# davidbau/rewriting

Hardware: NVIDIA H100
Metric: StyleGAN2-256 images/sec (higher is better)
Workload: dtype bf16x3 (3-term split bf16 operands, fp32 accumulate; fp32 in/out)

## Files before the change

### rewriting_b200/csrc/conv_tc.cu

```cuda
#include <cstdlib>
#include <cstring>

#include "rw_common.cuh"
#include "rw_kernels.h"

namespace rw {

namespace {

constexpr int BM = 128;
constexpr int BK = 32;
constexpr int MMA_K = 16;
constexpr int kStages = 7;
constexpr int kNumThreads = 384;
constexpr int kTmaWarp = 8;
constexpr uint32_t kProducerRegs = 40;
constexpr uint32_t kConsumerRegs = 232;
constexpr int kCluster = 2;
constexpr int kChunkKB = 16;

template <int BN>
struct ConvSmem {
  static constexpr int kABytes = BM * BK * 2;
  static constexpr int kBBytes = BN * BK * 2;
// ... 35 lines not shown

  const int m_tiles = (p.rows + BM - 1) / BM;
  const int n_tiles = p.Cout / BN;
  const int mn_units = (m_tiles + kCluster - 1) / kCluster * n_tiles;
  const int num_units = mn_units * p.nphase;
  const int kb_per_tap = p.Cin / BK;

  if (warp == kTmaWarp && lane == 0) {
    tma_prefetch_desc(&map_a_hi);
    tma_prefetch_desc(&map_a_lo);
    tma_prefetch_desc(&map_w_hi);
    tma_prefetch_desc(&map_w_lo);
    for (int s = 0; s < kStages; ++s) {
      mbar_init(&bars->full[s], 1);
      mbar_init(&bars->empty[s], 2 * kCluster);
    }
    fence_mbar_init();
  }
  cluster_sync();

  if (warp < kTmaWarp) {
    setmaxnreg_inc<kConsumerRegs>();
    const int wg = threadIdx.x >> 7;
    const int c = lane & 3;
    const int img = p.Hp * p.Wp;
    auto release = [&](int s) {
      if ((threadIdx.x & 127) == 0) {
#pragma unroll
        for (int r = 0; r < kCluster; ++r) mbar_arrive_cluster(mapa_shared(&bars->empty[s], r));
      }
    };
    auto clk = [] { return static_cast<uint32_t>(clock()); };
    uint32_t prof[6] = {0, 0, 0, 0, 0, 0};
    uint32_t tp0 = 0, tp1 = 0;
    if constexpr (PROF) prof[5] = 0u - clk();
    int stage = 0;
    uint32_t phase = 0;
    for (int unit = first_unit; unit < num_units; unit += nsched) {
      int ph, mn;
      decode_tile(unit, p.nphase, nsched, ph, mn);
      const int num_kb = p.ph_ntaps[ph] * kb_per_tap;
      const int n_tile = mn % n_tiles;
      const int n0 = n_tile * BN;
      const int m0 = ((mn / n_tiles) * kCluster + rank) * BM;

      float acc[NR], d[NR];
#pragma unroll
      for (int j = 0; j < NR; ++j) acc[j] = 0.f;
      for (int kb0 = 0; kb0 < num_kb; kb0 += kChunkKB) {
        const int kb_end = (kb0 + kChunkKB < num_kb) ? kb0 + kChunkKB : num_kb;
        int held = -1;
        for (int kb = kb0; kb < kb_end; ++kb) {
          if constexpr (PROF) tp0 = clk();
          mbar_wait(&bars->full[stage], phase);
          if constexpr (PROF) { tp1 = clk(); prof[0] += tp1 - tp0; }
          const uint32_t sa = smem_u32(smem + stage * S::kStageBytes);
          const uint64_t da_hi = make_smem_desc(sa + wg * (S::kABytes / 2), 16, 512, 2);
          const uint64_t da_lo = make_smem_desc(sa + S::kABytes + wg * (S::kABytes / 2), 16, 512, 2);
          const uint64_t db_hi = make_smem_desc(sa + 2 * S::kABytes, 16, 512, 2);
          const uint64_t db_lo = make_smem_desc(sa + 2 * S::kABytes + S::kBBytes, 16, 512, 2);
          wgmma_fence();
#pragma unroll
          for (int kk = 0; kk < BK / MMA_K; ++kk) {
            const uint64_t adv = static_cast<uint64_t>((kk * MMA_K * 2) >> 4);
            wgmma_m64nN<0, 0>(d, da_lo + adv, db_hi + adv, ((kb - kb0) | kk) != 0);
            wgmma_m64nN<0, 0>(d, da_hi + adv, db_lo + adv, 1u);
            wgmma_m64nN<0, 0>(d, da_hi + adv, db_hi + adv, 1u);
          }
          wgmma_commit();
          wgmma_wait<1>();
          if (held >= 0) release(held);
          held = stage;
          if (++stage == kStages) { stage = 0; phase ^= 1u; }
          if constexpr (PROF) prof[1] += clk() - tp1;
        }
        if constexpr (PROF) tp0 = clk();
        wgmma_wait<0>();
        release(held);
#pragma unroll
        for (int j = 0; j < NR; ++j) acc[j] += d[j];
        if constexpr (PROF) prof[2] += clk() - tp0;
      }
      if constexpr (PROF) tp0 = clk();

      uint32_t tid;
      asm volatile("mov.u32 %0, %%tid.x;\n" : "=r"(tid));
      const int row0 = m0 + ((tid >> 7) << 6) + (((tid >> 5) & 3) << 4) + ((tid & 31) >> 2);
#pragma unroll
      for (int i = 0; i < 2; ++i) {
        const int prow = row0 + 8 * i;
        const int b = prow / img;
        const int rem = prow - b * img;
        const int yy = rem / p.Wp;
        const int xx = rem - yy * p.Wp;
        const int Hv = p.ph_Hv[ph], Wv = p.ph_Wv[ph];
        const bool in_rows = prow < p.rows;
        const bool valid = in_rows && (yy < Hv) && (xx < Wv);
        const float* scl = (p.scale_bo && in_rows) ? p.scale_bo + static_cast<size_t>(b) * p.Cout : nullptr;
        float* outp = (p.out != nullptr && p.out_mode == 0 && valid)
                          ? p.out + p.ph_out_ofs[ph] + static_cast<size_t>(b) * p.out_sb +
                                static_cast<size_t>(yy) * p.out_sy + static_cast<size_t>(xx) * p.out_sx
                          : nullptr;
        if (EPI == 1 || !valid) {
          if (scl && (EPI == 1 || p.out_mode == 1)) {
#pragma unroll
            for (int j = 0; j < NJ; ++j) {
              const float2 sv = __ldg(reinterpret_cast<const float2*>(scl + n0 + 8 * j + 2 * c));
              acc[4 * j + 2 * i] *= sv.x;
              acc[4 * j + 2 * i + 1] *= sv.y;
            }
          }
          if (EPI == 1 && outp) {
#pragma unroll
            for (int j = 0; j < NJ; ++j)
#pragma unroll
              for (int e = 0; e < 2; ++e)
                outp[static_cast<size_t>(n0 + 8 * j + 2 * c + e) * p.out_sc] = acc[4 * j + 2 * i + e];
          }
        } else {
          float nz = 0.f;
          if (p.noise != nullptr)
            nz = __ldg(p.noise_w) * __ldg(p.noise + static_cast<size_t>(b) * p.noise_bstride +
                                          static_cast<size_t>(yy) * Wv + xx);
          const float act_gain = p.act_gain != 0.f ? p.act_gain : 1.4142135623730951f;
          if (scl) {
            const float* sc = scl + n0 + 2 * c;
#pragma unroll
            for (int j = 0; j < NJ; ++j)
#pragma unroll
              for (int e = 0; e < 2; ++e) acc[4 * j + 2 * i + e] *= __ldg(sc + 8 * j + e);
// ... 239 lines not shown
```

### rewriting_b200/csrc/rw_common.cuh

```cuda
#pragma once
#include <cuda_runtime.h>
#include <cuda_bf16.h>
#include <cuda.h>
#include <stdint.h>

namespace rw {

enum : int {
  RW_OK = 0,
  RW_ERR_BAD_ARG = -1,
  RW_ERR_CUDA = -2,
  RW_ERR_NO_DRIVER_SYMBOL = -3,
  RW_ERR_UNSUPPORTED = -4,
};
void set_last_error(const char* fmt, ...);
int check_cuda(cudaError_t e, const char* what);

#ifndef RW_SPIN_LIMIT
#define RW_SPIN_LIMIT (1u << 26)
#endif

__device__ __forceinline__ uint32_t smem_u32(const void* p) {
  return static_cast<uint32_t>(__cvta_generic_to_shared(p));
}

__device__ __forceinline__ uint32_t lane_id() { return threadIdx.x & 31u; }

__device__ __forceinline__ bool elect_one() {
  uint32_t pred = 0;
  asm volatile(
      "{\n\t.reg .pred P;\n\t"
      "elect.sync _|P, 0xffffffff;\n\t"
      "selp.u32 %0, 1, 0, P;\n\t}\n"
      : "=r"(pred));
  return pred != 0;
}

__device__ __forceinline__ void mbar_init(uint64_t* bar, uint32_t count) {
  asm volatile("mbarrier.init.shared::cta.b64 [%0], %1;\n" ::"r"(smem_u32(bar)), "r"(count));
}
__device__ __forceinline__ void fence_mbar_init() {
  asm volatile("fence.mbarrier_init.release.cluster;\n" ::: "memory");
}
__device__ __forceinline__ void fence_proxy_async_smem() {
  asm volatile("fence.proxy.async.shared::cta;\n" ::: "memory");
}
__device__ __forceinline__ void mbar_expect_tx(uint64_t* bar, uint32_t bytes) {
  asm volatile("mbarrier.arrive.expect_tx.shared::cta.b64 _, [%0], %1;\n" ::"r"(smem_u32(bar)),
               "r"(bytes)
               : "memory");
}
__device__ __forceinline__ void mbar_arrive(uint64_t* bar) {
  asm volatile("mbarrier.arrive.shared::cta.b64 _, [%0];\n" ::"r"(smem_u32(bar)) : "memory");
}
__device__ __forceinline__ bool mbar_try_wait(uint64_t* bar, uint32_t parity) {
  uint32_t ok;
  asm volatile(
      "{\n\t.reg .pred P;\n\t"
      "mbarrier.try_wait.parity.shared::cta.b64 P, [%1], %2;\n\t"
      "selp.u32 %0, 1, 0, P;\n\t}\n"
      : "=r"(ok)
      : "r"(smem_u32(bar)), "r"(parity)
      : "memory");
  return ok != 0;
}
__device__ __forceinline__ void mbar_wait(uint64_t* bar, uint32_t parity) {
  uint32_t spins = 0;
  while (!mbar_try_wait(bar, parity)) {
    if (++spins > RW_SPIN_LIMIT) __trap();
  }
}
__device__ __forceinline__ void named_bar_sync(int id, int count) {
  asm volatile("bar.sync %0, %1;\n" ::"r"(id), "r"(count) : "memory");
}

__device__ __forceinline__ uint32_t cluster_ctarank() {
  uint32_t r;
  asm volatile("mov.u32 %0, %%cluster_ctarank;\n" : "=r"(r));
  return r;
}
__device__ __forceinline__ uint32_t cluster_id_x() {
  uint32_t r;
  asm volatile("mov.u32 %0, %%clusterid.x;\n" : "=r"(r));
  return r;
}
__device__ __forceinline__ uint32_t num_clusters_x() {
  uint32_t r;
  asm volatile("mov.u32 %0, %%nclusterid.x;\n" : "=r"(r));
  return r;
}
__device__ __forceinline__ void cluster_sync() {
  asm volatile("barrier.cluster.arrive.release;\nbarrier.cluster.wait.acquire;\n" ::: "memory");
}
__device__ __forceinline__ uint32_t mapa_shared(const void* p, uint32_t rank) {
  uint32_t r;
  asm volatile("mapa.shared::cluster.u32 %0, %1, %2;\n" : "=r"(r) : "r"(smem_u32(p)), "r"(rank));
  return r;
}
__device__ __forceinline__ void mbar_arrive_cluster(uint32_t cluster_addr) {
  asm volatile("mbarrier.arrive.shared::cluster.b64 _, [%0];\n" ::"r"(cluster_addr) : "memory");
}

template <uint32_t N>
__device__ __forceinline__ void setmaxnreg_dec() {
  asm volatile("setmaxnreg.dec.sync.aligned.u32 %0;\n" ::"n"(N));
}
template <uint32_t N>
__device__ __forceinline__ void setmaxnreg_inc() {
  asm volatile("setmaxnreg.inc.sync.aligned.u32 %0;\n" ::"n"(N));
}

__device__ __forceinline__ void tma_prefetch_desc(const CUtensorMap* m) {
  asm volatile("prefetch.tensormap [%0];\n" ::"l"(reinterpret_cast<uint64_t>(m)) : "memory");
}
__device__ __forceinline__ void tma_load_2d(void* smem_dst, const CUtensorMap* m, uint64_t* bar,
                                            int32_t c_inner, int32_t c_outer) {
  asm volatile(
      "cp.async.bulk.tensor.2d.shared::cluster.global.mbarrier::complete_tx::bytes"
      " [%0], [%1, {%3, %4}], [%2];\n" ::"r"(smem_u32(smem_dst)),
      "l"(reinterpret_cast<uint64_t>(m)), "r"(smem_u32(bar)), "r"(c_inner), "r"(c_outer)
      : "memory");
}
__device__ __forceinline__ void tma_load_2d_multicast(void* smem_dst, const CUtensorMap* m,
                                                      uint64_t* bar, int32_t c_inner,
                                                      int32_t c_outer, uint16_t cta_mask) {
  asm volatile(
      "cp.async.bulk.tensor.2d.shared::cluster.global.mbarrier::complete_tx::bytes.multicast::cluster"
      " [%0], [%1, {%3, %4}], [%2], %5;\n" ::"r"(smem_u32(smem_dst)),
      "l"(reinterpret_cast<uint64_t>(m)), "r"(smem_u32(bar)), "r"(c_inner), "r"(c_outer),
      "h"(cta_mask)
      : "memory");
}

__device__ __forceinline__ void wgmma_fence() {
  asm volatile("wgmma.fence.sync.aligned;\n" ::: "memory");
}
__device__ __forceinline__ void wgmma_commit() {
  asm volatile("wgmma.commit_group.sync.aligned;\n" ::: "memory");
}
template <int N>
__device__ __forceinline__ void wgmma_wait() {
  asm volatile("wgmma.wait_group.sync.aligned %0;\n" ::"n"(N) : "memory");
}
template <int TA, int TB>
__device__ __forceinline__ void wgmma_m64n128(float (&d)[64], uint64_t desc_a, uint64_t desc_b,
                                               uint32_t accumulate) {
  asm volatile(
      "{\n\t.reg .pred p;\n\t"
      "setp.ne.b32 p, %66, 0;\n\t"
      "wgmma.mma_async.sync.aligned.m64n128k16.f32.bf16.bf16 "
      "{%0, %1, %2, %3, %4, %5, %6, %7, %8, %9, %10, %11, %12, %13, %14, %15, %16, %17, %18, %19, %20, %21, %22, %23, %24, %25, %26, %27, %28, %29, %30, %31, %32, %33, %34, %35, %36, %37, %38, %39, %40, %41, %42, %43, %44, %45, %46, %47, %48, %49, %50, %51, %52, %53, %54, %55, %56, %57, %58, %59, %60, %61, %62, %63}, "
      "%64, %65, p, 1, 1, %67, %68;\n\t}\n"
      : "+f"(d[0]), "+f"(d[1]), "+f"(d[2]), "+f"(d[3]), "+f"(d[4]), "+f"(d[5]), "+f"(d[6]), "+f"(d[7]),
        "+f"(d[8]), "+f"(d[9]), "+f"(d[10]), "+f"(d[11]), "+f"(d[12]), "+f"(d[13]), "+f"(d[14]), "+f"(d[15]),
        "+f"(d[16]), "+f"(d[17]), "+f"(d[18]), "+f"(d[19]), "+f"(d[20]), "+f"(d[21]), "+f"(d[22]), "+f"(d[23]),
        "+f"(d[24]), "+f"(d[25]), "+f"(d[26]), "+f"(d[27]), "+f"(d[28]), "+f"(d[29]), "+f"(d[30]), "+f"(d[31]),
        "+f"(d[32]), "+f"(d[33]), "+f"(d[34]), "+f"(d[35]), "+f"(d[36]), "+f"(d[37]), "+f"(d[38]), "+f"(d[39]),
        "+f"(d[40]), "+f"(d[41]), "+f"(d[42]), "+f"(d[43]), "+f"(d[44]), "+f"(d[45]), "+f"(d[46]), "+f"(d[47]),
        "+f"(d[48]), "+f"(d[49]), "+f"(d[50]), "+f"(d[51]), "+f"(d[52]), "+f"(d[53]), "+f"(d[54]), "+f"(d[55]),
        "+f"(d[56]), "+f"(d[57]), "+f"(d[58]), "+f"(d[59]), "+f"(d[60]), "+f"(d[61]), "+f"(d[62]), "+f"(d[63])
      : "l"(desc_a), "l"(desc_b), "r"(accumulate), "n"(TA), "n"(TB));
}
template <int TA, int TB>
__device__ __forceinline__ void wgmma_m64n64(float (&d)[32], uint64_t desc_a, uint64_t desc_b,
                                              uint32_t accumulate) {
  asm volatile(
      "{\n\t.reg .pred p;\n\t"
      "setp.ne.b32 p, %34, 0;\n\t"
      "wgmma.mma_async.sync.aligned.m64n64k16.f32.bf16.bf16 "
      "{%0, %1, %2, %3, %4, %5, %6, %7, %8, %9, %10, %11, %12, %13, %14, %15, %16, %17, %18, %19, %20, %21, %22, %23, %24, %25, %26, %27, %28, %29, %30, %31}, "
      "%32, %33, p, 1, 1, %35, %36;\n\t}\n"
      : "+f"(d[0]), "+f"(d[1]), "+f"(d[2]), "+f"(d[3]), "+f"(d[4]), "+f"(d[5]), "+f"(d[6]), "+f"(d[7]),
        "+f"(d[8]), "+f"(d[9]), "+f"(d[10]), "+f"(d[11]), "+f"(d[12]), "+f"(d[13]), "+f"(d[14]), "+f"(d[15]),
        "+f"(d[16]), "+f"(d[17]), "+f"(d[18]), "+f"(d[19]), "+f"(d[20]), "+f"(d[21]), "+f"(d[22]), "+f"(d[23]),
        "+f"(d[24]), "+f"(d[25]), "+f"(d[26]), "+f"(d[27]), "+f"(d[28]), "+f"(d[29]), "+f"(d[30]), "+f"(d[31])
      : "l"(desc_a), "l"(desc_b), "r"(accumulate), "n"(TA), "n"(TB));
}
template <int TA, int TB, int NR>
__device__ __forceinline__ void wgmma_m64nN(float (&d)[NR], uint64_t desc_a, uint64_t desc_b,
                                             uint32_t accumulate) {
  static_assert(NR == 64 || NR == 32, "wgmma_m64nN: N = 128 or 64");
  if constexpr (NR == 64) wgmma_m64n128<TA, TB>(d, desc_a, desc_b, accumulate);
  else wgmma_m64n64<TA, TB>(d, desc_a, desc_b, accumulate);
}
template <int TA, int TB>
__device__ __forceinline__ void wgmma_m64n144(float (&d)[72], uint64_t desc_a, uint64_t desc_b,
                                               uint32_t accumulate) {
  asm volatile(
      "{\n\t.reg .pred p;\n\t"
      "setp.ne.b32 p, %74, 0;\n\t"
      "wgmma.mma_async.sync.aligned.m64n144k16.f32.bf16.bf16 "
      "{%0, %1, %2, %3, %4, %5, %6, %7, %8, %9, %10, %11, %12, %13, %14, %15, %16, %17, %18, %19, %20, %21, %22, %23, %24, %25, %26, %27, %28, %29, %30, %31, %32, %33, %34, %35, %36, %37, %38, %39, %40, %41, %42, %43, %44, %45, %46, %47, %48, %49, %50, %51, %52, %53, %54, %55, %56, %57, %58, %59, %60, %61, %62, %63, %64, %65, %66, %67, %68, %69, %70, %71}, "
      "%72, %73, p, 1, 1, %75, %76;\n\t}\n"
      : "+f"(d[0]), "+f"(d[1]), "+f"(d[2]), "+f"(d[3]), "+f"(d[4]), "+f"(d[5]), "+f"(d[6]), "+f"(d[7]),
        "+f"(d[8]), "+f"(d[9]), "+f"(d[10]), "+f"(d[11]), "+f"(d[12]), "+f"(d[13]), "+f"(d[14]), "+f"(d[15]),
// ... 35 lines not shown
```

### rewriting_b200/csrc/upconv_tc.cu

```cuda
#include <cstring>

#include "rw_common.cuh"
#include "rw_kernels.h"

namespace rw {

namespace {

constexpr int UM = 128;
constexpr int UNC = 16;
constexpr int UN = 9 * UNC;
constexpr int UBK = 32;
constexpr int UK = 16;
constexpr int kUStages = 5;
constexpr int kUThreads = 384;
constexpr int kUTmaWarp = 8;
constexpr uint32_t kUProducerRegs = 40;
constexpr uint32_t kUConsumerRegs = 232;
constexpr int kUABytes = UM * UBK * 2;
constexpr int kUBBytes = UN * UBK * 2;
constexpr int kUStageBytes = 2 * kUABytes + 2 * kUBBytes;
constexpr int kUMailFloats = 2 * 2 * 4 * 2 * 32;
constexpr int kUOutSlotBytes = 64 * 32;
constexpr int kUOutQuarterBytes = 2 * kUOutSlotBytes;
constexpr int kUOutStageBytes = 4 * kUOutQuarterBytes;
constexpr int kUXchgFloat2 = 9 * 2 * 32;
constexpr int kUXchgBytes = 8 * kUXchgFloat2 * 8;
constexpr int kUSmemTotal =
    kUStages * kUStageBytes + kUMailFloats * 4 + kUOutStageBytes + kUXchgBytes + 512 + 256;
static_assert(kUSmemTotal <= 232448, "upconv_fused: shared memory over the per-block limit");

struct UBarriers {
  uint64_t full[kUStages];
  uint64_t empty[kUStages];
};

__device__ __forceinline__ void tma_load_5d(void* smem_dst, const CUtensorMap* m, uint64_t* bar,
                                            int32_t c0, int32_t c1, int32_t c2, int32_t c3,
                                            int32_t c4) {
  asm volatile(
      "cp.async.bulk.tensor.5d.shared::cluster.global.mbarrier::complete_tx::bytes"
      " [%0], [%1, {%3, %4, %5, %6, %7}], [%2];\n" ::"r"(smem_u32(smem_dst)),
      "l"(reinterpret_cast<uint64_t>(m)), "r"(smem_u32(bar)), "r"(c0), "r"(c1), "r"(c2), "r"(c3),
      "r"(c4)
      : "memory");
}

__device__ __forceinline__ float2 f2add(float2 a, float2 b) {
  return make_float2(__fadd_rn(a.x, b.x), __fadd_rn(a.y, b.y));
}
__device__ __forceinline__ float2 f2mul(float2 a, float2 b) {
  return make_float2(__fmul_rn(a.x, b.x), __fmul_rn(a.y, b.y));
}
__device__ __forceinline__ float2 f2fma(float2 a, float2 b, float2 c) {
  return make_float2(__fmaf_rn(a.x, b.x, c.x), __fmaf_rn(a.y, b.y, c.y));
}
__device__ __forceinline__ void mbar_wait_relaxed(uint64_t* bar, uint32_t parity) {
  uint32_t spins = 0;
  while (!mbar_try_wait(bar, parity)) {
    __nanosleep(40);
    if (++spins > RW_SPIN_LIMIT) __trap();
  }
}

__device__ __forceinline__ void sts_v4(uint32_t a, float x, float y, float z, float w) {
  asm volatile("st.shared.v4.f32 [%0], {%1, %2, %3, %4};\n" ::"r"(a), "f"(x), "f"(y), "f"(z), "f"(w)
               : "memory");
}
__device__ __forceinline__ void lds_v4(uint32_t a, float& x, float& y, float& z, float& w) {
  asm volatile("ld.shared.v4.f32 {%0, %1, %2, %3}, [%4];\n"
               : "=f"(x), "=f"(y), "=f"(z), "=f"(w)
               : "r"(a)
               : "memory");
}

constexpr int kBarPair = 3;
template <int N>
__device__ __forceinline__ void tma_store_wait_read_n() {
  asm volatile("cp.async.bulk.wait_group.read %0;\n" ::"n"(N) : "memory");
}

struct UpItem {
  int bg, band, cg;
  int y_first, y_emit, y_end;
};

__device__ __forceinline__ UpItem decode_item(int item, const UpFusedParams& p) {
  UpItem it;
  it.cg = item % p.ncg;
  const int r = item / p.ncg;
  it.band = r % p.nbands;
  it.bg = r / p.nbands;
  const int ya = 1 + (it.band * p.H) / p.nbands;
  const int yb = 1 + ((it.band + 1) * p.H) / p.nbands;
  it.y_emit = ya;
  it.y_first = ya - 2 < 0 ? 0 : ya - 2;
  it.y_end = yb;
  return it;
}

__device__ __forceinline__ void stmatrix_x4(uint32_t addr, const uint32_t (&r)[4]) {
  asm volatile("stmatrix.sync.aligned.m8n8.x4.shared.b16 [%0], {%1, %2, %3, %4};\n" ::"r"(addr),
               "r"(r[0]), "r"(r[1]), "r"(r[2]), "r"(r[3])
               : "memory");
}

__device__ __forceinline__ void tma_store_5d(const CUtensorMap* m, uint32_t smem_src, int32_t c0,
                                             int32_t c1, int32_t c2, int32_t c3, int32_t c4) {
  asm volatile(
      "cp.async.bulk.tensor.5d.global.shared::cta.bulk_group [%0, {%2, %3, %4, %5, %6}], [%1];\n" ::"l"(
          reinterpret_cast<uint64_t>(m)),
      "r"(smem_src), "r"(c0), "r"(c1), "r"(c2), "r"(c3), "r"(c4)
      : "memory");
  asm volatile("cp.async.bulk.commit_group;\n" ::: "memory");
}
__device__ __forceinline__ void tma_store_wait_all() {
  asm volatile("cp.async.bulk.wait_group 0;\n" ::: "memory");
}

template <bool PROF, bool NCHW>
__global__ void __launch_bounds__(kUThreads, 1)
upconv_fused_kernel(const __grid_constant__ CUtensorMap map_a_hi,
                    const __grid_constant__ CUtensorMap map_a_lo,
                    const __grid_constant__ CUtensorMap map_w_hi,
                    const __grid_constant__ CUtensorMap map_w_lo,
                    const __grid_constant__ CUtensorMap map_o_hi,
                    const __grid_constant__ CUtensorMap map_o_lo, const UpFusedParams p) {
  extern __shared__ uint8_t smem_raw[];
  uint8_t* smem = reinterpret_cast<uint8_t*>((reinterpret_cast<uintptr_t>(smem_raw) + 511) &
                                             ~static_cast<uintptr_t>(511));
  float* mail = reinterpret_cast<float*>(smem + kUStages * kUStageBytes);
  uint8_t* out_stage = smem + kUStages * kUStageBytes + kUMailFloats * 4;
  float2* xchg = reinterpret_cast<float2*>(out_stage + kUOutStageBytes);
  UBarriers* bars = reinterpret_cast<UBarriers*>(out_stage + kUOutStageBytes + kUXchgBytes);

  const int warp = __shfl_sync(0xffffffffu, static_cast<int>(threadIdx.x >> 5), 0);
  const int lane = threadIdx.x & 31;
  const int kb_count = p.Cin / UBK;
  const int G = UM / p.W;

  if (warp == kUTmaWarp && lane == 0) {
    tma_prefetch_desc(&map_a_hi);
    tma_prefetch_desc(&map_a_lo);
    tma_prefetch_desc(&map_w_hi);
    tma_prefetch_desc(&map_w_lo);
    tma_prefetch_desc(&map_o_hi);
    tma_prefetch_desc(&map_o_lo);
    for (int s = 0; s < kUStages; ++s) {
      mbar_init(&bars->full[s], 1);
      mbar_init(&bars->empty[s], 2);
    }
    fence_mbar_init();
  }
  __syncthreads();

  if (warp < kUTmaWarp) {
    setmaxnreg_inc<kUConsumerRegs>();
    const int wg = warp >> 2;
    const int q = warp >> 1;
    const int h = warp & 1;
    int stage = 0;
    uint32_t phase = 0;
    const int g = lane >> 2, c = lane & 3;
    const int W = p.W;
    const int T0 = q * 32 + 4 * g;
    const int x0 = T0 & (W - 1);
    const int img_in_tile = T0 / W;
    const int Ho = 2 * p.H, Wo = 2 * W;
    const bool first_x = (x0 == 0), last_x = (x0 + 4 == W);
    const bool cross = W > 32;
    const bool mail_l = cross && g == 0 && !first_x, mail_r = cross && g == 7 && !last_x;
    float kv[4], kh[4];
    {
      const float k00 = __ldg(p.k4 + 15);
#pragma unroll
      for (int a = 0; a < 4; ++a) {
        kv[a] = __ldg(p.k4 + 15 - a * 4);
        kh[a] = __ldg(p.k4 + 15 - a) / k00;
      }
    }
    const float nw = (!NCHW || (p.noise != nullptr && p.noise_w != nullptr)) ? __ldg(p.noise_w) : 0.f;
    uint32_t step = 0;
    constexpr uint32_t kMailBufBytes = 2 * 4 * 2 * 32 * 4;
    const uint32_t mail_s = smem_u32(mail) + h * (4 * 2 * 32 * 4) + c * 32;
    const uint32_t post_r = mail_s + (q * 2 + 1) * 128, post_l = mail_s + (q * 2 + 0) * 128;
    const uint32_t read_l = mail_s + ((q - 1) * 2 + 1) * 128, read_r = mail_s + ((q + 1) * 2 + 0) * 128;
    const uint32_t slot_s = smem_u32(out_stage) + q * kUOutQuarterBytes;
    uint32_t st_addr[2];
    {
      const int m = lane >> 3, gp = lane & 7;
      const int Wm = W < 32 ? W : 32;
      const int tl = 4 * gp + m;
      const int il = tl / W;
      const int xg = ((4 * gp) & (Wm - 1)) >> 2;
#pragma unroll
      for (int xi = 0; xi < 2; ++xi) {
        uint32_t a = slot_s + (((il * 8 + 2 * m + xi) * (Wm >> 2) + xg) << 5) + (h << 4);
        a ^= ((a >> 7) & 1u) << 4;
        st_addr[xi] = a;
      }
    }
    const CUtensorMap* omap = h ? &map_o_lo : &map_o_hi;
    const uint32_t my_slot = slot_s + h * kUOutSlotBytes;
    const int o_xg = ((32 * q) & (W - 1)) >> 2;
    const int o_img = (32 * q) / W;
    long long prof_acc[16] = {0, 0, 0, 0, 0, 0, 0, 0, 0, 0, 0, 0, 0, 0, 0, 0};

    for (int item = blockIdx.x; item < p.nitems; item += gridDim.x) {
      const UpItem it = decode_item(item, p);
      const int b0 = it.bg * G;
      const int b = b0 + img_in_tile;
      const bool img_ok = b < p.B;
      const int c0 = it.cg * UNC + h * 8 + 2 * c;
      const size_t chan_o = static_cast<size_t>(img_ok ? b : 0) * p.Cout + c0;
      float2 dm = make_float2(1.f, 1.f), bs = make_float2(0.f, 0.f), ns = make_float2(1.f, 1.f);
      if (!NCHW || p.demod != nullptr) dm = __ldg(reinterpret_cast<const float2*>(p.demod + chan_o));
      if (!NCHW || (p.act && p.bias != nullptr)) bs = __ldg(reinterpret_cast<const float2*>(p.bias + c0));
      if (!NCHW) ns = __ldg(reinterpret_cast<const float2*>(p.next_scale + chan_o));
      const bool has_noise = !NCHW || (p.noise != nullptr && p.noise_w != nullptr);
      float2 c20[4], c21[4], c22[4];
      float2 w0[2][4], w1[2][4], w2[2][4];
#pragma unroll
      for (int j = 0; j < 4; ++j) {
        c20[j] = c21[j] = c22[j] = make_float2(0.f, 0.f);
        w0[0][j] = w0[1][j] = w1[0][j] = w1[1][j] = w2[0][j] = w2[1][j] = make_float2(0.f, 0.f);
      }
      const float* nrow_base = p.noise + static_cast<size_t>(img_ok ? b : 0) * p.noise_bstride + 2 * x0;
      __nv_bfloat16* out_hi = static_cast<__nv_bfloat16*>(p.next_hi);
      __nv_bfloat16* out_lo = static_cast<__nv_bfloat16*>(p.next_lo);
      const size_t img_row0 = static_cast<size_t>(img_ok ? b : 0) * (Ho + 1);

      for (int y = it.y_first; y < it.y_end; ++y, ++step) {
        const bool rows_out = (y >= it.y_emit);
        const bool emit = rows_out && img_ok;
        if (emit && c < 2 && has_noise) {
          const float* np = nrow_base + static_cast<size_t>(2 * y - 2 + c) * Wo;
          asm volatile("prefetch.global.L1 [%0];\n" ::"l"(np));
        }
        long long tq[8];
        if constexpr (PROF) tq[0] = clock64();
        float2 P[9][4];
        {
          float d[72];
          int held = -1;
          for (int kb = 0; kb < kb_count; ++kb) {
            mbar_wait(&bars->full[stage], phase);
            const uint32_t sa = smem_u32(smem + stage * kUStageBytes);
            const uint64_t da_hi = make_smem_desc(sa + wg * (kUABytes / 2), 16, 512, 2);
            const uint64_t da_lo = make_smem_desc(sa + kUABytes + wg * (kUABytes / 2), 16, 512, 2);
            const uint64_t db_hi = make_smem_desc(sa + 2 * kUABytes, 16, 512, 2);
            const uint64_t db_lo = make_smem_desc(sa + 2 * kUABytes + kUBBytes, 16, 512, 2);
            wgmma_fence();
#pragma unroll
            for (int kk = 0; kk < UBK / UK; ++kk) {
              const uint64_t adv = static_cast<uint64_t>((kk * UK * 2) >> 4);
              wgmma_m64n144<0, 0>(d, da_lo + adv, db_hi + adv, (kb | kk) != 0);
              wgmma_m64n144<0, 0>(d, da_hi + adv, db_lo + adv, 1u);
              wgmma_m64n144<0, 0>(d, da_hi + adv, db_hi + adv, 1u);
            }
            wgmma_commit();
            wgmma_wait<1>();
            if (held >= 0 && (threadIdx.x & 127) == 0) mbar_arrive(&bars->empty[held]);
            held = stage;
            if (++stage == kUStages) { stage = 0; phase ^= 1u; }
          }
          wgmma_wait<0>();
          if ((threadIdx.x & 127) == 0) mbar_arrive(&bars->empty[held]);
          if constexpr (PROF) tq[1] = clock64();
          float2* to = xchg + (warp ^ 1) * kUXchgFloat2 + lane;
#pragma unroll
          for (int t = 0; t < 9; ++t)
#pragma unroll
            for (int i = 0; i < 2; ++i)
              to[(t * 2 + i) * 32] = h ? make_float2(d[4 * t + 2 * i], d[4 * t + 2 * i + 1])
                                       : make_float2(d[4 * (9 + t) + 2 * i], d[4 * (9 + t) + 2 * i + 1]);
          named_bar_sync(kBarPair + q, 64);
          const float2* from = xchg + warp * kUXchgFloat2 + lane;
#pragma unroll
          for (int t = 0; t < 9; ++t)
#pragma unroll
            for (int i = 0; i < 2; ++i) {
              const float2 own = h ? make_float2(d[4 * (9 + t) + 2 * i], d[4 * (9 + t) + 2 * i + 1])
                                   : make_float2(d[4 * t + 2 * i], d[4 * t + 2 * i + 1]);
              const float2 other = from[(t * 2 + i) * 32];
              P[t][i] = h ? other : own;
              P[t][2 + i] = h ? own : other;
            }
          named_bar_sync(kBarPair + q, 64);
        }
        if constexpr (PROF) tq[2] = clock64();
        if (p.debug_p != nullptr && img_ok && y < p.H && y >= it.y_emit - 1) {
#pragma unroll
          for (int j = 0; j < 4; ++j) {
            float* dp = p.debug_p + ((static_cast<size_t>(b) * p.H + y) * W + x0 + j) * 9 * p.Cout + c0;
#pragma unroll
            for (int t = 0; t < 9; ++t) *reinterpret_cast<float2*>(dp + t * p.Cout) = P[t][j];
          }
        }

        float2 le[2][4], ro[2][4], od[2][4];
#pragma unroll
        for (int j = 0; j < 4; ++j) {
          le[0][j] = f2add(P[0][j], c20[j]);
          od[0][j] = f2add(P[1][j], c21[j]);
          ro[0][j] = f2add(P[2][j], c22[j]);
          le[1][j] = P[3][j];
          od[1][j] = P[4][j];
          ro[1][j] = P[5][j];
          c20[j] = P[6][j];
          c21[j] = P[7][j];
          c22[j] = P[8][j];
        }
        const uint32_t mbo = (step & 1u) * kMailBufBytes;
        if (cross) {
          if (g == 7) {
            sts_v4(post_r + mbo, ro[0][3].x, ro[0][3].y, od[0][3].x, od[0][3].y);
            sts_v4(post_r + mbo + 16, ro[1][3].x, ro[1][3].y, od[1][3].x, od[1][3].y);
          }
          if (g == 0) {
            sts_v4(post_l + mbo, le[0][0].x, le[0][0].y, od[0][0].x, od[0][0].y);
// ... 75 lines not shown
                const float nzv = nw * nz[2 * j + xi];
                float2 v;
                if (yi == 0)
                  v = f2fma(kv3, hf[0][xi][j],
                                 f2fma(kv2, w2[xi][j], f2fma(kv1, w1[xi][j], f2mul(kv0, w0[xi][j]))));
                else
                  v = f2fma(kv3, hf[1][xi][j],
                                 f2fma(kv2, hf[0][xi][j], f2fma(kv1, w2[xi][j], f2mul(kv0, w1[xi][j]))));
                v = f2add(f2fma(v, dm, make_float2(nzv, nzv)), bs);
                if (!NCHW || p.act) {
                  const float2 t02 = f2mul(v, make_float2(0.2f, 0.2f));
                  v = f2mul(make_float2(fmaxf(v.x, t02.x), fmaxf(v.y, t02.y)),
                                 make_float2(1.4142135623730951f, 1.4142135623730951f));
                }
                if constexpr (NCHW) {
                  yv[xi][j] = v;
                } else {
                  const float2 kk = f2mul(ns, v);
                  const __nv_bfloat162 hh = __floats2bfloat162_rn(kk.x, kk.y);
                  const uint32_t hu = *reinterpret_cast<const uint32_t*>(&hh);
                  const __nv_bfloat162 ll = __floats2bfloat162_rn(
                      kk.x - __uint_as_float(hu << 16), kk.y - __uint_as_float(hu & 0xffff0000u));
                  hw[xi][j] = hu;
                  lw[xi][j] = *reinterpret_cast<const uint32_t*>(&ll);
                }
              }
            }
            if constexpr (NCHW) {
              if (img_ok) {
                float* yrow = p.y_out + ((static_cast<size_t>(b) * p.Cout + c0) * Ho + Y) * Wo + 2 * x0;
                const size_t cstride = static_cast<size_t>(Ho) * Wo;
                *reinterpret_cast<float4*>(yrow) = make_float4(yv[0][0].x, yv[1][0].x, yv[0][1].x, yv[1][1].x);
                *reinterpret_cast<float4*>(yrow + 4) = make_float4(yv[0][2].x, yv[1][2].x, yv[0][3].x, yv[1][3].x);
                *reinterpret_cast<float4*>(yrow + cstride) = make_float4(yv[0][0].y, yv[1][0].y, yv[0][1].y, yv[1][1].y);
                *reinterpret_cast<float4*>(yrow + cstride + 4) =
                    make_float4(yv[0][2].y, yv[1][2].y, yv[0][3].y, yv[1][3].y);
              }
              continue;
            }
            if constexpr (PROF) te[1] = clock64();
            if (lane == 0) tma_store_wait_read_n<0>();
            named_bar_sync(kBarPair + q, 64);
            if constexpr (PROF) te[2] = clock64();
#pragma unroll
            for (int xi = 0; xi < 2; ++xi) {
              stmatrix_x4(st_addr[xi], hw[xi]);
              stmatrix_x4(st_addr[xi] + kUOutSlotBytes, lw[xi]);
            }
            if constexpr (PROF) te[5] = clock64();
            fence_proxy_async_smem();
            if constexpr (PROF) te[6] = clock64();
            named_bar_sync(kBarPair + q, 64);
            if constexpr (PROF) te[3] = clock64();
            if (lane == 0 && (!PROF || p.debug_nostore == 0))
              tma_store_5d(omap, my_slot, it.cg * UNC, o_xg, 0, Y, b0 + o_img);
            if constexpr (PROF) {
              te[4] = clock64();
#pragma unroll
              for (int i = 0; i < 4; ++i) prof_acc[8 + i] += te[i + 1] - te[i];
              prof_acc[12] += te[5] - te[2];
              prof_acc[13] += te[6] - te[5];
              prof_acc[14] += te[3] - te[6];
            }
            if (img_ok && last_x && c == 0) {
              const size_t off = ((img_row0 + Y) * (Wo + 1) + Wo) * p.Cout + it.cg * UNC + h * 8;
              *reinterpret_cast<uint4*>(out_hi + off) = make_uint4(0u, 0u, 0u, 0u);
              *reinterpret_cast<uint4*>(out_lo + off) = make_uint4(0u, 0u, 0u, 0u);
            }
          }
        }
        if (!NCHW && emit && y == p.H) {
          const size_t prow = (img_row0 + Ho) * (Wo + 1);
#pragma unroll
          for (int i = 0; i < 3; ++i) {
            if (i < 2 || (last_x && c == 3)) {
              const size_t off = (prow + 2 * x0 + 2 * c + i) * p.Cout + it.cg * UNC + h * 8;
              *reinterpret_cast<uint4*>(out_hi + off) = make_uint4(0u, 0u, 0u, 0u);
              *reinterpret_cast<uint4*>(out_lo + off) = make_uint4(0u, 0u, 0u, 0u);
            }
          }
        }
        if constexpr (PROF) {
          tq[5] = clock64();
          prof_acc[0] += tq[1] - tq[0];
          prof_acc[1] += tq[2] - tq[1];
          prof_acc[2] += tq[3] - tq[2];
          prof_acc[3] += tq[6] - tq[3];
          prof_acc[4] += tq[7] - tq[6];
          prof_acc[5] += tq[4] - tq[7];
          prof_acc[6] += tq[5] - tq[4];
          prof_acc[7] += 1;
        }
#pragma unroll
        for (int xi = 0; xi < 2; ++xi)
#pragma unroll
          for (int j = 0; j < 4; ++j) {
            w0[xi][j] = w2[xi][j];
            w1[xi][j] = hf[0][xi][j];
            w2[xi][j] = hf[1][xi][j];
          }
      }
    }
    if (!NCHW && lane == 0) tma_store_wait_all();
    if constexpr (PROF) {
      if (lane == 0 && p.debug_prof != nullptr) {
        long long* dst = p.debug_prof + (static_cast<size_t>(blockIdx.x) * 8 + warp) * 16;
#pragma unroll
        for (int i = 0; i < 16; ++i) dst[i] = prof_acc[i];
      }
    }
  } else {
    setmaxnreg_dec<kUProducerRegs>();
    if (warp != kUTmaWarp) return;
    int stage = 0;
    uint32_t phase = 0;
    const bool wide = p.W >= 32;
    const int nop = wide ? G : 4;
    const int plane = lane / nop, idx = lane % nop;
    const CUtensorMap* amap = plane ? &map_a_lo : &map_a_hi;
    const CUtensorMap* wmap = (lane & 1) ? &map_w_lo : &map_w_hi;
    const uint32_t a_off = plane * kUABytes + idx * (kUABytes / nop);
    for (int item = blockIdx.x; item < p.nitems; item += gridDim.x) {
      const UpItem it = decode_item(item, p);
      const int b0 = it.bg * G;
      const int wrow = it.cg * UN;
      for (int y = it.y_first; y < it.y_end; ++y) {
        for (int kb = 0; kb < kb_count; ++kb) {
          if (lane == 0) {
            mbar_wait_relaxed(&bars->empty[stage], phase ^ 1u);
            mbar_expect_tx(&bars->full[stage], kUStageBytes);
          }
          __syncwarp();
          uint8_t* st = smem + stage * kUStageBytes;
          if (lane < 2 * nop) {
            if (wide)
              tma_load_5d(st + a_off, amap, &bars->full[stage], kb * UBK, 0, 0, 0,
                          (b0 + idx) * (p.H + 1) + y);
            else
              tma_load_5d(st + a_off, amap, &bars->full[stage], kb * UBK, 0, b0 + idx * (32 / p.W), 0, y);
          } else if (lane >= 30) {
            tma_load_2d(st + 2 * kUABytes + (lane & 1) * kUBBytes, wmap, &bars->full[stage], kb * UBK,
                        wrow);
          }
          if (++stage == kUStages) { stage = 0; phase ^= 1u; }
        }
      }
    }
    return;
  }

}

}

int make_tmap_nd_bf16(CUtensorMap* out, const void* base, int rank, const uint64_t* dims,
                      const uint64_t* strides_bytes, const uint32_t* box, const uint32_t* estrides,
                      int swizzle);

int upconv_fused_launch(const UpFusedParams& pin, const void* a_hi, const void* a_lo,
                        const void* w_hi, const void* w_lo, cudaStream_t stream) {
  UpFusedParams p = pin;
  const int W = p.W, H = p.H;
  if (W < 4 || W > UM || (W & (W - 1)) != 0 || H < 1 || p.Cin % UBK != 0 || p.Cout % UNC != 0 ||
      p.B < 1) {
    set_last_error("upconv_fused: unsupported shape B=%d Cin=%d Cout=%d H=%d W=%d", p.B, p.Cin,
                   p.Cout, H, W);
    return RW_ERR_BAD_ARG;
  }
  const int G = UM / W;
  const int nbg = (p.B + G - 1) / G;
  p.ncg = p.Cout / UNC;
  const int sms = device_sm_count();
  int best = 1;
  long long best_cost = -1;
  for (int nb = 1; nb <= 32 && H / nb >= 4; nb *= 2) {
    const long long items = static_cast<long long>(nbg) * p.ncg * nb;
    const long long waves = (items + sms - 1) / sms;
    const long long cost = waves * ((H + nb - 1) / nb + 2);
    if (best_cost < 0 || cost < best_cost) {
      best_cost = cost;
      best = nb;
    }
  }
  p.nbands = best;
  p.nitems = nbg * p.ncg * p.nbands;

  CUtensorMap ma_hi, ma_lo, mw_hi, mw_lo, mo_hi, mo_lo;
  const uint32_t Wm = W < 32 ? W : 32;
  const uint64_t kpx = static_cast<uint64_t>(p.Cin) * 2;
  const uint64_t krow = static_cast<uint64_t>(W + 1) * kpx;
  int rc;
  if (W >= 32) {
    const uint64_t dims[5] = {static_cast<uint64_t>(p.Cin), 8, 4, static_cast<uint64_t>(W / 32),
                              static_cast<uint64_t>(p.B) * (H + 1)};
    const uint64_t str[4] = {4 * kpx, kpx, 32 * kpx, krow};
    const uint32_t box[5] = {UBK, 8u, 4u, static_cast<uint32_t>(W / 32), 1u};
    if ((rc = make_tmap_nd_bf16(&ma_hi, a_hi, 5, dims, str, box, nullptr, 3))) return rc;
    if ((rc = make_tmap_nd_bf16(&ma_lo, a_lo, 5, dims, str, box, nullptr, 3))) return rc;
  } else {
    const uint64_t dims[5] = {static_cast<uint64_t>(p.Cin), static_cast<uint64_t>(W / 4),
                              static_cast<uint64_t>(p.B), 4, static_cast<uint64_t>(H + 1)};
    const uint64_t str[4] = {4 * kpx, static_cast<uint64_t>(H + 1) * krow, kpx, krow};
    const uint32_t box[5] = {UBK, static_cast<uint32_t>(W / 4), 32u / Wm, 4u, 1u};
    if ((rc = make_tmap_nd_bf16(&ma_hi, a_hi, 5, dims, str, box, nullptr, 3))) return rc;
    if ((rc = make_tmap_nd_bf16(&ma_lo, a_lo, 5, dims, str, box, nullptr, 3))) return rc;
  }
  if (p.y_out == nullptr) {
    const uint64_t Wo = 2 * static_cast<uint64_t>(W), Ho = 2 * static_cast<uint64_t>(H);
    const uint64_t px = static_cast<uint64_t>(p.Cout) * 2;
    const uint64_t od[5] = {static_cast<uint64_t>(p.Cout), Wo / 8, 8, Ho + 1, static_cast<uint64_t>(p.B)};
    const uint64_t os[4] = {8 * px, px, (Wo + 1) * px, (Ho + 1) * (Wo + 1) * px};
    const uint32_t ob[5] = {UNC, Wm / 4, 8u, 1u, 32u / Wm};
    if ((rc = make_tmap_nd_bf16(&mo_hi, p.next_hi, 5, od, os, ob, nullptr, 1))) return rc;
    if ((rc = make_tmap_nd_bf16(&mo_lo, p.next_lo, 5, od, os, ob, nullptr, 1))) return rc;
  } else {
    if ((reinterpret_cast<uintptr_t>(p.y_out) & 15u) != 0) {
      set_last_error("upconv_fused: y must be 16-byte aligned");
      return RW_ERR_BAD_ARG;
    }
    mo_hi = ma_hi;
    mo_lo = ma_lo;
  }
  const uint64_t wdims[2] = {static_cast<uint64_t>(p.Cin), static_cast<uint64_t>(p.ncg) * UN};
  const uint64_t wstr[1] = {static_cast<uint64_t>(p.Cin) * 2};
  const uint32_t wbox[2] = {UBK, UN};
  if ((rc = make_tmap_nd_bf16(&mw_hi, w_hi, 2, wdims, wstr, wbox, nullptr, 3))) return rc;
  if ((rc = make_tmap_nd_bf16(&mw_lo, w_lo, 2, wdims, wstr, wbox, nullptr, 3))) return rc;
  const int grid = p.nitems < sms ? p.nitems : sms;
  auto launch = [&](auto kernel, bool& attr_done) -> int {
    if (!attr_done) {
      int e = check_cuda(cudaFuncSetAttribute(kernel, cudaFuncAttributeMaxDynamicSharedMemorySize,
                                              kUSmemTotal),
                         "upconv_fused smem attr");
      if (e) return e;
      attr_done = true;
    }
    kernel<<<grid, kUThreads, kUSmemTotal, stream>>>(ma_hi, ma_lo, mw_hi, mw_lo, mo_hi, mo_lo, p);
    return check_cuda(cudaGetLastError(), "upconv_fused launch");
  };
  static bool attr_prof = false, attr_planes = false, attr_nchw = false;
  if (p.debug_prof != nullptr) return launch(upconv_fused_kernel<true, false>, attr_prof);
  if (p.y_out != nullptr) return launch(upconv_fused_kernel<false, true>, attr_nchw);
  return launch(upconv_fused_kernel<false, false>, attr_planes);
}

}
```

Baseline: 1937.

## Launch upconv kernel as 2-CTA clusters with multicast TMA for activation tiles

After: 1931, median of 6. About the same (-0.3%).

```diff
diff --git a/rewriting_b200/csrc/conv_tc.cu b/rewriting_b200/csrc/conv_tc.cu
--- a/rewriting_b200/csrc/conv_tc.cu
+++ b/rewriting_b200/csrc/conv_tc.cu
@@ -111,7 +111,7 @@
         int held = -1;
         for (int kb = kb0; kb < kb_end; ++kb) {
           if constexpr (PROF) tp0 = clk();
-          mbar_wait(&bars->full[stage], phase);
+          mbar_wait_mma(&bars->full[stage], phase);
           if constexpr (PROF) { tp1 = clk(); prof[0] += tp1 - tp0; }
           const uint32_t sa = smem_u32(smem + stage * S::kStageBytes);
           const uint64_t da_hi = make_smem_desc(sa + wg * (S::kABytes / 2), 16, 512, 2);
@@ -135,6 +135,7 @@
         }
         if constexpr (PROF) tp0 = clk();
         wgmma_wait<0>();
+        wgmma_fence_operands(d);
         release(held);
 #pragma unroll
         for (int j = 0; j < NR; ++j) acc[j] += d[j];
diff --git a/rewriting_b200/csrc/rw_common.cuh b/rewriting_b200/csrc/rw_common.cuh
--- a/rewriting_b200/csrc/rw_common.cuh
+++ b/rewriting_b200/csrc/rw_common.cuh
@@ -70,6 +70,15 @@
     if (++spins > RW_SPIN_LIMIT) __trap();
   }
 }
+__device__ __forceinline__ void mbar_wait_mma(uint64_t* bar, uint32_t parity) {
+  uint32_t spins = 0;
+  while (!mbar_try_wait(bar, parity)) {
+    if (++spins > RW_SPIN_LIMIT) {
+      asm volatile("wgmma.wait_group.sync.aligned 0;\n" ::: "memory");
+      __trap();
+    }
+  }
+}
 __device__ __forceinline__ void named_bar_sync(int id, int count) {
   asm volatile("bar.sync %0, %1;\n" ::"r"(id), "r"(count) : "memory");
 }
@@ -141,6 +150,11 @@
 template <int N>
 __device__ __forceinline__ void wgmma_wait() {
   asm volatile("wgmma.wait_group.sync.aligned %0;\n" ::"n"(N) : "memory");
+}
+template <int NR>
+__device__ __forceinline__ void wgmma_fence_operands(float (&d)[NR]) {
+#pragma unroll
+  for (int i = 0; i < NR; ++i) asm volatile("" : "+f"(d[i])::"memory");
 }
 template <int TA, int TB>
 __device__ __forceinline__ void wgmma_m64n128(float (&d)[64], uint64_t desc_a, uint64_t desc_b,
diff --git a/rewriting_b200/csrc/upconv_tc.cu b/rewriting_b200/csrc/upconv_tc.cu
--- a/rewriting_b200/csrc/upconv_tc.cu
+++ b/rewriting_b200/csrc/upconv_tc.cu
@@ -15,6 +15,7 @@
 constexpr int kUStages = 5;
 constexpr int kUThreads = 384;
 constexpr int kUTmaWarp = 8;
+constexpr int kUCluster = 2;
 constexpr uint32_t kUProducerRegs = 40;
 constexpr uint32_t kUConsumerRegs = 232;
 constexpr int kUABytes = UM * UBK * 2;
@@ -35,14 +36,14 @@
   uint64_t empty[kUStages];
 };
 
-__device__ __forceinline__ void tma_load_5d(void* smem_dst, const CUtensorMap* m, uint64_t* bar,
-                                            int32_t c0, int32_t c1, int32_t c2, int32_t c3,
-                                            int32_t c4) {
+__device__ __forceinline__ void tma_load_5d_multicast(void* smem_dst, const CUtensorMap* m,
+                                                      uint64_t* bar, int32_t c0, int32_t c1,
+                                                      int32_t c2, int32_t c3, int32_t c4) {
   asm volatile(
-      "cp.async.bulk.tensor.5d.shared::cluster.global.mbarrier::complete_tx::bytes"
-      " [%0], [%1, {%3, %4, %5, %6, %7}], [%2];\n" ::"r"(smem_u32(smem_dst)),
+      "cp.async.bulk.tensor.5d.shared::cluster.global.mbarrier::complete_tx::bytes.multicast::cluster"
+      " [%0], [%1, {%3, %4, %5, %6, %7}], [%2], %8;\n" ::"r"(smem_u32(smem_dst)),
       "l"(reinterpret_cast<uint64_t>(m)), "r"(smem_u32(bar)), "r"(c0), "r"(c1), "r"(c2), "r"(c3),
-      "r"(c4)
+      "r"(c4), "h"(static_cast<uint16_t>((1u << kUCluster) - 1))
       : "memory");
 }
 
@@ -82,13 +83,16 @@
 
 struct UpItem {
   int bg, band, cg;
+  bool cg_ok;
   int y_first, y_emit, y_end;
 };
 
-__device__ __forceinline__ UpItem decode_item(int item, const UpFusedParams& p) {
+__device__ __forceinline__ UpItem decode_item(int item, int rank, const UpFusedParams& p) {
   UpItem it;
-  it.cg = item % p.ncg;
-  const int r = item / p.ncg;
+  const int npair = (p.ncg + kUCluster - 1) / kUCluster;
+  it.cg = (item % npair) * kUCluster + rank;
+  it.cg_ok = it.cg < p.ncg;
+  const int r = item / npair;
   it.band = r % p.nbands;
   it.bg = r / p.nbands;
   const int ya = 1 + (it.band * p.H) / p.nbands;
@@ -138,6 +142,9 @@
   const int lane = threadIdx.x & 31;
   const int kb_count = p.Cin / UBK;
   const int G = UM / p.W;
+  const int rank = static_cast<int>(cluster_ctarank());
+  const int nsched = static_cast<int>(num_clusters_x());
+  const int first_item = static_cast<int>(cluster_id_x());
 
   if (warp == kUTmaWarp && lane == 0) {
     tma_prefetch_desc(&map_a_hi);
@@ -148,11 +155,11 @@
     tma_prefetch_desc(&map_o_lo);
     for (int s = 0; s < kUStages; ++s) {
       mbar_init(&bars->full[s], 1);
-      mbar_init(&bars->empty[s], 2);
+      mbar_init(&bars->empty[s], 2 * kUCluster);
     }
     fence_mbar_init();
   }
-  __syncthreads();
+  cluster_sync();
 
   if (warp < kUTmaWarp) {
     setmaxnreg_inc<kUConsumerRegs>();
@@ -204,14 +211,20 @@
     const uint32_t my_slot = slot_s + h * kUOutSlotBytes;
     const int o_xg = ((32 * q) & (W - 1)) >> 2;
     const int o_img = (32 * q) / W;
+    auto release = [&](int s) {
+      if ((threadIdx.x & 127) == 0) {
+#pragma unroll
+        for (int r = 0; r < kUCluster; ++r) mbar_arrive_cluster(mapa_shared(&bars->empty[s], r));
+      }
+    };
     long long prof_acc[16] = {0, 0, 0, 0, 0, 0, 0, 0, 0, 0, 0, 0, 0, 0, 0, 0};
 
-    for (int item = blockIdx.x; item < p.nitems; item += gridDim.x) {
-      const UpItem it = decode_item(item, p);
+    for (int item = first_item; item < p.nitems; item += nsched) {
+      const UpItem it = decode_item(item, rank, p);
       const int b0 = it.bg * G;
       const int b = b0 + img_in_tile;
-      const bool img_ok = b < p.B;
-      const int c0 = it.cg * UNC + h * 8 + 2 * c;
+      const bool img_ok = b < p.B && it.cg_ok;
+      const int c0 = (it.cg_ok ? it.cg : 0) * UNC + h * 8 + 2 * c;
       const size_t chan_o = static_cast<size_t>(img_ok ? b : 0) * p.Cout + c0;
       float2 dm = make_float2(1.f, 1.f), bs = make_float2(0.f, 0.f), ns = make_float2(1.f, 1.f);
       if (!NCHW || p.demod != nullptr) dm = __ldg(reinterpret_cast<const float2*>(p.demod + chan_o));
@@ -244,7 +257,7 @@
           float d[72];
           int held = -1;
           for (int kb = 0; kb < kb_count; ++kb) {
-            mbar_wait(&bars->full[stage], phase);
+            mbar_wait_mma(&bars->full[stage], phase);
             const uint32_t sa = smem_u32(smem + stage * kUStageBytes);
             const uint64_t da_hi = make_smem_desc(sa + wg * (kUABytes / 2), 16, 512, 2);
             const uint64_t da_lo = make_smem_desc(sa + kUABytes + wg * (kUABytes / 2), 16, 512, 2);
@@ -260,12 +273,13 @@
             }
             wgmma_commit();
             wgmma_wait<1>();
-            if (held >= 0 && (threadIdx.x & 127) == 0) mbar_arrive(&bars->empty[held]);
+            if (held >= 0) release(held);
             held = stage;
             if (++stage == kUStages) { stage = 0; phase ^= 1u; }
           }
           wgmma_wait<0>();
-          if ((threadIdx.x & 127) == 0) mbar_arrive(&bars->empty[held]);
+          wgmma_fence_operands(d);
+          release(held);
           if constexpr (PROF) tq[1] = clock64();
           float2* to = xchg + (warp ^ 1) * kUXchgFloat2 + lane;
 #pragma unroll
@@ -447,7 +461,7 @@
             if constexpr (PROF) te[6] = clock64();
             named_bar_sync(kBarPair + q, 64);
             if constexpr (PROF) te[3] = clock64();
-            if (lane == 0 && (!PROF || p.debug_nostore == 0))
+            if (lane == 0 && it.cg_ok && (!PROF || p.debug_nostore == 0))
               tma_store_5d(omap, my_slot, it.cg * UNC, o_xg, 0, Y, b0 + o_img);
             if constexpr (PROF) {
               te[4] = clock64();
@@ -506,7 +520,7 @@
     }
   } else {
     setmaxnreg_dec<kUProducerRegs>();
-    if (warp != kUTmaWarp) return;
+    if (warp == kUTmaWarp) {
     int stage = 0;
     uint32_t phase = 0;
     const bool wide = p.W >= 32;
@@ -515,8 +529,8 @@
     const CUtensorMap* amap = plane ? &map_a_lo : &map_a_hi;
     const CUtensorMap* wmap = (lane & 1) ? &map_w_lo : &map_w_hi;
     const uint32_t a_off = plane * kUABytes + idx * (kUABytes / nop);
-    for (int item = blockIdx.x; item < p.nitems; item += gridDim.x) {
-      const UpItem it = decode_item(item, p);
+    for (int item = first_item; item < p.nitems; item += nsched) {
+      const UpItem it = decode_item(item, rank, p);
       const int b0 = it.bg * G;
       const int wrow = it.cg * UN;
       for (int y = it.y_first; y < it.y_end; ++y) {
@@ -528,11 +542,14 @@
           __syncwarp();
           uint8_t* st = smem + stage * kUStageBytes;
           if (lane < 2 * nop) {
-            if (wide)
-              tma_load_5d(st + a_off, amap, &bars->full[stage], kb * UBK, 0, 0, 0,
-                          (b0 + idx) * (p.H + 1) + y);
-            else
-              tma_load_5d(st + a_off, amap, &bars->full[stage], kb * UBK, 0, b0 + idx * (32 / p.W), 0, y);
+            if (plane == rank) {
+              if (wide)
+                tma_load_5d_multicast(st + a_off, amap, &bars->full[stage], kb * UBK, 0, 0, 0,
+                                      (b0 + idx) * (p.H + 1) + y);
+              else
+                tma_load_5d_multicast(st + a_off, amap, &bars->full[stage], kb * UBK, 0,
+                                      b0 + idx * (32 / p.W), 0, y);
+            }
           } else if (lane >= 30) {
             tma_load_2d(st + 2 * kUABytes + (lane & 1) * kUBBytes, wmap, &bars->full[stage], kb * UBK,
                         wrow);
@@ -541,9 +558,9 @@
         }
       }
     }
-    return;
-  }
-
+    }
+  }
+  cluster_sync();
 }
 
 }
@@ -565,12 +582,43 @@
   const int G = UM / W;
   const int nbg = (p.B + G - 1) / G;
   p.ncg = p.Cout / UNC;
-  const int sms = device_sm_count();
+  const int npair = (p.ncg + kUCluster - 1) / kUCluster;
+  auto kernel = p.debug_prof != nullptr ? upconv_fused_kernel<true, false>
+              : p.y_out != nullptr      ? upconv_fused_kernel<false, true>
+                                        : upconv_fused_kernel<false, false>;
+  const int kv = p.debug_prof != nullptr ? 0 : p.y_out != nullptr ? 1 : 2;
+  cudaLaunchConfig_t cfg = {};
+  cudaLaunchAttribute attr[1];
+  attr[0].id = cudaLaunchAttributeClusterDimension;
+  attr[0].val.clusterDim.x = kUCluster;
+  attr[0].val.clusterDim.y = 1;
+  attr[0].val.clusterDim.z = 1;
+  cfg.blockDim = dim3(kUThreads);
+  cfg.dynamicSmemBytes = kUSmemTotal;
+  cfg.stream = stream;
+  cfg.attrs = attr;
+  cfg.numAttrs = 1;
+  static int max_clusters[3] = {0, 0, 0};
+  if (max_clusters[kv] == 0) {
+    int e = check_cuda(cudaFuncSetAttribute(kernel, cudaFuncAttributeMaxDynamicSharedMemorySize,
+                                            kUSmemTotal),
+                       "upconv_fused smem attr");
+    if (e) return e;
+    cfg.gridDim = dim3(kUCluster * (device_sm_count() / kUCluster));
+    e = check_cuda(cudaOccupancyMaxActiveClusters(&max_clusters[kv], kernel, &cfg),
+                   "upconv_fused cluster occupancy");
+    if (e) return e;
+    if (max_clusters[kv] < 1) {
+      set_last_error("upconv_fused: no cluster of %d CTAs fits on the device", kUCluster);
+      return RW_ERR_UNSUPPORTED;
+    }
+  }
+  const int slots = max_clusters[kv];
   int best = 1;
   long long best_cost = -1;
   for (int nb = 1; nb <= 32 && H / nb >= 4; nb *= 2) {
-    const long long items = static_cast<long long>(nbg) * p.ncg * nb;
-    const long long waves = (items + sms - 1) / sms;
+    const long long items = static_cast<long long>(nbg) * npair * nb;
+    const long long waves = (items + slots - 1) / slots;
     const long long cost = waves * ((H + nb - 1) / nb + 2);
     if (best_cost < 0 || cost < best_cost) {
       best_cost = cost;
@@ -578,7 +626,7 @@
     }
   }
   p.nbands = best;
-  p.nitems = nbg * p.ncg * p.nbands;
+  p.nitems = nbg * npair * p.nbands;
 
   CUtensorMap ma_hi, ma_lo, mw_hi, mw_lo, mo_hi, mo_lo;
   const uint32_t Wm = W < 32 ? W : 32;
@@ -621,22 +669,12 @@
   const uint32_t wbox[2] = {UBK, UN};
   if ((rc = make_tmap_nd_bf16(&mw_hi, w_hi, 2, wdims, wstr, wbox, nullptr, 3))) return rc;
   if ((rc = make_tmap_nd_bf16(&mw_lo, w_lo, 2, wdims, wstr, wbox, nullptr, 3))) return rc;
-  const int grid = p.nitems < sms ? p.nitems : sms;
-  auto launch = [&](auto kernel, bool& attr_done) -> int {
-    if (!attr_done) {
-      int e = check_cuda(cudaFuncSetAttribute(kernel, cudaFuncAttributeMaxDynamicSharedMemorySize,
-                                              kUSmemTotal),
-                         "upconv_fused smem attr");
-      if (e) return e;
-      attr_done = true;
-    }
-    kernel<<<grid, kUThreads, kUSmemTotal, stream>>>(ma_hi, ma_lo, mw_hi, mw_lo, mo_hi, mo_lo, p);
-    return check_cuda(cudaGetLastError(), "upconv_fused launch");
-  };
-  static bool attr_prof = false, attr_planes = false, attr_nchw = false;
-  if (p.debug_prof != nullptr) return launch(upconv_fused_kernel<true, false>, attr_prof);
-  if (p.y_out != nullptr) return launch(upconv_fused_kernel<false, true>, attr_nchw);
-  return launch(upconv_fused_kernel<false, false>, attr_planes);
-}
-
-}
+  const int clusters = p.nitems < slots ? p.nitems : slots;
+  cfg.gridDim = dim3(kUCluster * clusters);
+  if ((rc = check_cuda(cudaLaunchKernelEx(&cfg, kernel, ma_hi, ma_lo, mw_hi, mw_lo, mo_hi, mo_lo, p),
+                       "upconv_fused launch")))
+    return rc;
+  return check_cuda(cudaGetLastError(), "upconv_fused launch");
+}
+
+}
```
